# liuliu/ccv

Measured on AMD Instinct MI355X. Metric: images/sec fwd+bwd VGG-D 224x224 bs256, higher is better.
Workload: dtype f32 (Winograd-domain / fc GEMMs: exact bf16x3 split, all 9 products, fp32 accumulate); 1 GPU; VGG-D (ccv vgg_d_params, 225x225x3 crop, NHWC) forward+backward+SGD, batch 256 per GPU, random-init weights; global_batch=256, parallelism=dp1, conv_relu=convolution epilogue (NNC_MI355X_CONV_ALGO_FUSE_RELU)

## Files before the change

### ccv_amd/csrc/cmd_conv.cpp

```cpp
#include "gemm_launch.h"
#include "winograd.h"
#include "wino_fused.h"
#include "wino_wgrad_fused.h"
#include "conv_c3.h"

using namespace nnc;

namespace {

static size_t align256(size_t x) { return (x + 255) & ~(size_t)255; }

static thread_local int tl_relu_want = 0, tl_relu_done = 0;
static thread_local int tl_mask_want = 0, tl_mask_done = 0;
static thread_local Image4 tl_mask = { 0, 0, 0, 0, 0, 0, 0, 0, 0 };
static bool mask_fits(const Image4& dst)
{
	const Image4& m = tl_mask;
	return m.p && m.n == dst.n && m.h == dst.h && m.w == dst.w && m.c == dst.c && m.sc == 1 && aligned16(m.p) && m.sw % 4 == 0 && m.sh % 4 == 0 && (m.n == 1 || m.sn % 4 == 0);
}

struct back_share_t {
	int want_v;
	int want_bits;
	int GYn, GXn, KB;
	float* v;
	unsigned* bits;
	size_t v_off, bits_off;
};
static thread_local back_share_t tl_share = { 0, 0, 0, 0, 0, 0, 0, 0, 0 };

static void* g_dbg_bits_dst = 0;
static size_t g_dbg_bits_cap = 0, g_dbg_bits_got = 0;
static long g_back_shared[2] = { 0, 0 };

struct conv_geom_t {
	int N, H, W, C;
	int OH, OW, K;
	int kh, kw, Cg, Kg, groups;
	int sy, sx, pby, pbx, dy, dx;
};

static bool conv_geometry(const ccv_nnc_cmd_t& cmd, const ccv_nnc_hint_t& hint, const Image4& a, const Image4& b, const ccv_nnc_tensor_t* w, conv_geom_t* g)
{
	g->N = a.n; g->H = a.h; g->W = a.w; g->C = a.c;
	g->OH = b.h; g->OW = b.w; g->K = b.c;
	g->groups = cmd.info.convolution.groups > 0 ? cmd.info.convolution.groups : 1;
	g->kh = cmd.info.size.dim[0]; g->kw = cmd.info.size.dim[1];
	if (g->K != cmd.info.convolution.count || g->K % g->groups || g->C % g->groups || a.n != b.n) return false;
	g->Cg = g->C / g->groups; g->Kg = g->K / g->groups;
	g->sy = hint.stride.dim[0] > 0 ? hint.stride.dim[0] : 1;
	g->sx = hint.stride.dim[1] > 0 ? hint.stride.dim[1] : 1;
	g->pby = hint.border.begin[0]; g->pbx = hint.border.begin[1];
	g->dy = cmd.info.convolution.dilation[0] > 1 ? cmd.info.convolution.dilation[0] : 1;
	g->dx = cmd.info.convolution.dilation[1] > 1 ? cmd.info.convolution.dilation[1] : 1;
	(void)w;
	return true;
// ... 40 lines not shown
}

static int wino_slice_images(const int N, const int tiles_per_image, const int C_src, const int C_dst)
{
	const long kb = tune(TUNE_WINO_SLICE_KB);
	if (kb <= 0) return N;
	const double per_image = 36.0 * sizeof(float) * (double)tiles_per_image * (double)(C_src + C_dst);
	long nb = (long)((double)kb * 1024.0 / per_image);
	if (nb < 1) nb = 1;
	return nb > N ? N : (int)nb;
}

template <bool FLIP>
static int conv_wino_run(const char* name, const conv_geom_t& g, const wino_plan_t& p, const Image4& src, const float* w, const float* bias, const Image4& dst, const int pad_y, const int pad_x, const int flags, ccv_nnc_stream_context_t* const ctx)
{
	const int Cs = src.c, Cd = dst.c;
	const int per_image = p.TH * p.TW;
	const int nb = wino_slice_images(g.N, per_image, Cs, Cd);
	const size_t v_bytes = nb == g.N ? p.v_bytes : (sizeof(float) * 36 * (size_t)nb * per_image * Cs + 255) & ~(size_t)255;
	const size_t m_bytes = nb == g.N ? p.m_bytes : (sizeof(float) * 36 * (size_t)nb * per_image * Cd + 255) & ~(size_t)255;
	bool have_v = FLIP && tl_share.v && nb == g.N && p.u_bytes + m_bytes <= tl_share.v_off;
	size_t need = p.u_bytes + v_bytes + m_bytes;
	if (have_v && tl_share.v_off + v_bytes > need) need = tl_share.v_off + v_bytes;
	char* ws = (char*)workspace_of(ctx, need);
	if (!ws) return CCV_NNC_EXEC_OOM;
	if (have_v && (float*)(ws + tl_share.v_off) != tl_share.v) have_v = false;
	float* const U = (float*)ws;
	float* const V = have_v ? tl_share.v : (float*)(ws + p.u_bytes);
	float* const M = have_v ? (float*)(ws + p.u_bytes) : (float*)(ws + p.u_bytes + v_bytes);
	hipStream_t stream = stream_of(ctx);
	hipLaunchKernelGGL(HIP_KERNEL_NAME(wino_weight_kernel<FLIP>), dim3(blocks_exact((size_t)Cs * Cd, 256)), dim3(256), 0, stream, w, U, g.K, g.C);
	HIP_ENFORCE(hipGetLastError());
	for (int n0 = 0; n0 < g.N; n0 += nb) {
		const int ns = g.N - n0 < nb ? g.N - n0 : nb;
		const int T = ns * per_image;
		WinoTiles ti;
		ti.TH = p.TH; ti.TW = p.TW; ti.T = T;
		ti.H = src.h; ti.W = src.w; ti.sn = src.sn; ti.sh = src.sh; ti.sw = src.sw; ti.oy = -pad_y; ti.ox = -pad_x; ti.C4 = Cs / 4;
		ti.relu = (!FLIP && tl_relu_want) ? 1 : 0;
		if (ti.relu) tl_relu_done = 1;
		ti.mask = 0; ti.m_sn = ti.m_sh = ti.m_sw = 0;
		ti.d_c4.init(ti.C4); ti.d_tw.init(ti.TW); ti.d_th.init(ti.TH);
		if (!have_v) hipLaunchKernelGGL(HIP_KERNEL_NAME(wino_input_kernel<false>), dim3(blocks_exact((size_t)T * ti.C4, 256)), dim3(256), 0, stream, (const float*)src.p + (long)n0 * src.sn, V, ti, WinoMaskOut());
		HIP_ENFORCE(hipGetLastError());
		MatLoader<true, true> la, lb;
		la.p = V; la.ldr = Cs; la.ldk = 1; la.R = T; la.K = Cs;
		lb.p = U; lb.ldr = Cs; lb.ldk = 1; lb.R = Cd; lb.K = Cs;
		GemmOut out = { M, Cd, 1, 0, 1.f, 0 };
		const int ret = gemm_run(name, la, lb, out, T, Cd, Cs, 36, (long)T * Cs, (long)Cd * Cs, (long)T * Cd, 0L, 1, flags, ctx);
		if (ret != CCV_NNC_EXEC_SUCCESS) return ret;
		ti.H = dst.h; ti.W = dst.w; ti.sn = dst.sn; ti.sh = dst.sh; ti.sw = dst.sw; ti.C4 = Cd / 4;
		ti.d_c4.init(ti.C4);
		if (FLIP && mask_fits(dst)) {
			ti.mask = tl_mask.p + (long)n0 * tl_mask.sn; ti.m_sn = tl_mask.sn; ti.m_sh = tl_mask.sh; ti.m_sw = tl_mask.sw;
			tl_mask_done = 1;
		}
		hipLaunchKernelGGL(wino_output_kernel, dim3(blocks_exact((size_t)T * ti.C4, 256)), dim3(256), 0, stream, (const float*)M, bias, dst.p + (long)n0 * dst.sn, ti);
		HIP_ENFORCE(hipGetLastError());
	}
	return CCV_NNC_EXEC_SUCCESS;
}

struct wino_fused_plan_t {
	int GH, GW, GYn, GXn, groups, KB, CCn;
	size_t uf_bytes;
};

static bool wino_fused_plan(const conv_geom_t& g, const Image4& src, const Image4& dst, wino_fused_plan_t* p)
{
	if (g.kh != 3 || g.kw != 3 || g.sy != 1 || g.sx != 1 || g.dy != 1 || g.dx != 1 || g.groups != 1) return false;
	if (src.c % WF_CC || src.c < 2 * WF_CC || src.sc != 1 || dst.sc != 1 || !aligned16(src.p) || src.sw % 4 || src.sh % 4 || (src.n > 1 && src.sn % 4)) return false;
	if (dst.c % 4 || !aligned16(dst.p) || dst.sw % 4 || dst.sh % 4 || (dst.n > 1 && dst.sn % 4)) return false;
	if (((long)(dst.h - 1) * dst.sh + (long)(dst.w - 1) * dst.sw + dst.c) * 4 >= (long)WF_OOB) return false;
	if (((long)(src.h - 1) * src.sh + (long)(src.w - 1) * src.sw + src.c) * 4 >= (long)WF_OOB) return false;
	const int TH = (dst.h + 3) / 4, TW = (dst.w + 3) / 4;
	static const int shapes[3][2] = { { 4, 4 }, { 2, 8 }, { 8, 2 } };
	long best = -1;
	for (int i = 0; i < 3; i++) {
		const long cover = (long)((TH + shapes[i][0] - 1) / shapes[i][0]) * ((TW + shapes[i][1] - 1) / shapes[i][1]);
		if (best < 0 || cover < best) { best = cover; p->GH = shapes[i][0]; p->GW = shapes[i][1]; }
// ... 111 lines not shown
	const long tiles = (long)((g.K + 127) / 128) * ((g.C + 127) / 128) * 36;
	long s = ((long)device_cu_count() * 8 + tiles - 1) / tiles;
	const long max_s = p->t.T / (GEMM_BK * 8);
	if (s > max_s) s = max_s;
	if (s > 64) s = 64;
	p->splits = s <= 1 ? 1 : (int)(((s < 8 ? 8 : s) + 7) & ~7);
	p->w_bytes = p->t.m_bytes;
	p->du_bytes = (sizeof(float) * 36 * (size_t)g.K * g.C + 255) & ~(size_t)255;
	p->head_bytes = p->splits > 1 ? sizeof(float) * 36 * (size_t)g.K * g.C * p->splits : 0;
	const size_t colsum_bound = sizeof(float) * (size_t)device_cu_count() * 4 * g.K;
	if (p->head_bytes < colsum_bound) p->head_bytes = colsum_bound;
	p->head_bytes = (p->head_bytes + 255) & ~(size_t)255;
	p->blocks = ((long)p->t.T * (g.K / 4) + 255) / 256;
	p->bp_bytes = sizeof(float) * (size_t)p->blocks * g.K;
	return true;
}

static int conv_wino_wgrad(const conv_geom_t& g, const wino_wgrad_plan_t& p, const Image4& gr, const Image4& a, float* dw, float* dbias, bool* bias_done, const int flags, ccv_nnc_stream_context_t* const ctx)
{
	const int per_image = p.t.TH * p.t.TW;
	const int nb = wino_slice_images(g.N, per_image, g.C, g.K);
	const size_t bits_bytes = (size_t)g.N * tl_share.GYn * tl_share.GXn * tl_share.KB * 1024;
	const bool fuse_bias = dbias && 256 % (g.K / 4) == 0;
	const size_t extra = nb != g.N ? 0 : (tl_share.want_v ? (fuse_bias ? p.w_bytes : 0) : (tl_share.want_bits ? bits_bytes : 0));
	char* ws = (char*)workspace_of(ctx, p.total() + extra);
	if (!ws) return CCV_NNC_EXEC_OOM;
	float* const Vg = extra && tl_share.want_v ? (float*)(ws + p.total()) : 0;
	unsigned* const bits = extra && tl_share.want_bits ? (unsigned*)(ws + p.total()) : 0;
	float* const V = (float*)(ws + p.head_bytes);
	float* const W = (float*)(ws + p.head_bytes + p.t.v_bytes);
	float* const dU = (float*)(ws + p.head_bytes + p.t.v_bytes + p.w_bytes);
	float* const BP = (float*)(ws + p.head_bytes + p.t.v_bytes + p.w_bytes + p.du_bytes);
	const int acc = (flags & CCV_NNC_ACCUMULATE_OUTPUT) ? 1 : 0;
	hipStream_t stream = stream_of(ctx);
	if (bits && (tl_share.GYn * 2 != p.t.TH || tl_share.GXn * 8 != p.t.TW || g.C % WF_KT)) {
		const int r = fill_f32((float*)bits, bits_bytes / sizeof(float), 0.f, ctx);
		if (r != CCV_NNC_EXEC_SUCCESS) return r;
	}
	for (int n0 = 0; n0 < g.N; n0 += nb) {
		const int ns = g.N - n0 < nb ? g.N - n0 : nb;
		const int T = ns * per_image;
		WinoTiles ti;
		ti.TH = p.t.TH; ti.TW = p.t.TW; ti.T = T;
		ti.H = a.h; ti.W = a.w; ti.sn = a.sn; ti.sh = a.sh; ti.sw = a.sw; ti.oy = -g.pby; ti.ox = -g.pbx; ti.C4 = g.C / 4;
		ti.d_c4.init(ti.C4); ti.d_tw.init(ti.TW); ti.d_th.init(ti.TH);
		if (bits) {
			WinoMaskOut mo;
			mo.bits = (unsigned char*)bits; mo.GYn = tl_share.GYn; mo.GXn = tl_share.GXn; mo.KB = tl_share.KB;
			hipLaunchKernelGGL(HIP_KERNEL_NAME(wino_input_kernel<true>), dim3(blocks_exact((size_t)T * ti.C4, 256)), dim3(256), 0, stream, (const float*)a.p + (long)n0 * a.sn, V, ti, mo);
			tl_share.bits = bits; tl_share.bits_off = p.total();
			__atomic_fetch_add(&g_back_shared[1], 1L, __ATOMIC_RELAXED);
		} else hipLaunchKernelGGL(HIP_KERNEL_NAME(wino_input_kernel<false>), dim3(blocks_exact((size_t)T * ti.C4, 256)), dim3(256), 0, stream, (const float*)a.p + (long)n0 * a.sn, V, ti, WinoMaskOut());
		HIP_ENFORCE(hipGetLastError());
		ti.H = gr.h; ti.W = gr.w; ti.sn = gr.sn; ti.sh = gr.sh; ti.sw = gr.sw; ti.oy = 0; ti.ox = 0; ti.C4 = g.K / 4;
		ti.d_c4.init(ti.C4);
		const long blocks = ((long)T * (g.K / 4) + 255) / 256;
		const float* const grs = (const float*)gr.p + (long)n0 * gr.sn;
		if (Vg) {
			ti.oy = -1; ti.ox = -1;
			hipLaunchKernelGGL(wino_outgrad_both_kernel, dim3((unsigned)blocks), dim3(256), 0, stream, grs, Vg, W, ti, BP);
			tl_share.v = Vg; tl_share.v_off = p.total();
			__atomic_fetch_add(&g_back_shared[0], 1L, __ATOMIC_RELAXED);
		} else if (fuse_bias) hipLaunchKernelGGL(HIP_KERNEL_NAME(wino_outgrad_kernel<true>), dim3((unsigned)blocks), dim3(256), 0, stream, grs, W, ti, BP);
		else hipLaunchKernelGGL(HIP_KERNEL_NAME(wino_outgrad_kernel<false>), dim3((unsigned)blocks), dim3(256), 0, stream, grs, W, ti, (float*)0);
		HIP_ENFORCE(hipGetLastError());
		MatLoader<false, true> la, lb;
		la.p = W; la.ldr = 1; la.ldk = g.K; la.R = g.K; la.K = T;
		lb.p = V; lb.ldr = 1; lb.ldk = g.C; lb.R = g.C; lb.K = T;
		GemmOut out = { dU, g.C, 1, 0, 1.f, n0 > 0 ? 1 : 0 };
		int splits = p.splits;
		if (nb < g.N) {
			const long max_s = T / (GEMM_BK * 8);
			if (splits > max_s) splits = max_s <= 1 ? 1 : (int)(max_s & ~7L);
			if (splits < 8) splits = 1;
		}
// ... 262 lines not shown
				const int r = conv_forw_nhwc(q, gr, Fw, 0, ti, CONV_ALGO_IMPLICIT_GEMM, flags & ~CCV_NNC_ACCUMULATE_OUTPUT, ctx);
				if (r != CCV_NNC_EXEC_SUCCESS) return r;
			}
			hipLaunchKernelGGL(parity_scatter_kernel, dim3(grid_for(cells, 256)), dim3(256), 0, stream, (const float*)T, h.p, U, V, vec ? g.C / 4 : -g.C, h.sn, h.sh, h.sw, py, px, cells);
			HIP_ENFORCE(hipGetLastError());
		}
	return CCV_NNC_EXEC_SUCCESS;
}

static bool conv_dgrad_takes_fused(const conv_geom_t& g, const Image4& gr, const Image4& h, const int algo, wino_fused_plan_t* fp)
{
	return algo != CONV_ALGO_IMPLICIT_GEMM && algo != CONV_ALGO_WINOGRAD && g.pby <= 2 && g.pbx <= 2 && g.pby >= 0 && g.pbx >= 0 && wino_fused_plan(g, gr, h, fp) && (algo == CONV_ALGO_WINOGRAD_FUSED || wino_fused_preferred(g.K, *fp, h));
}
static bool conv_dgrad_takes_wino(const conv_geom_t& g, const Image4& gr, const float* w, const Image4& h, const int algo, wino_plan_t* wp)
{
	return algo != CONV_ALGO_IMPLICIT_GEMM && wino_plan(g, g.H, g.W, g.K, g.C, wp) && wino_images_ok(gr, h, w, 0) && (algo >= CONV_ALGO_WINOGRAD || wino_preferred(*wp, g.K, g.C));
}

static int conv_dgrad_nhwc(const conv_geom_t& g, const Image4& gr, const float* w, const Image4& h, const int algo, const int flags, ccv_nnc_stream_context_t* const ctx)
{
	if (gr.sc != 1 || !pixel_linear(h) || !image_fits_int(gr)) return CCV_NNC_EXEC_INVALID;
	wino_plan_t wp;
	wino_fused_plan_t fp;
	if (conv_dgrad_takes_fused(g, gr, h, algo, &fp)) {
		const int r = conv_wino_fused_run<true>("conv_dgrad_wino_fused", g, fp, gr, w, 0, h, 2 - g.pby, 2 - g.pbx, ctx);
		if (r != CCV_NNC_EXEC_OOM) return r;
	}
	if (conv_dgrad_takes_wino(g, gr, w, h, algo, &wp)) {
		const int r = conv_wino_run<true>("conv_dgrad_wino", g, wp, gr, w, 0, h, 2 - g.pby, 2 - g.pbx, flags, ctx);
		if (r != CCV_NNC_EXEC_OOM) return r;
	}
	if (algo != CONV_ALGO_IMPLICIT_GEMM && !(flags & CCV_NNC_ACCUMULATE_OUTPUT) && conv_dgrad_parity_ok(g) && g.kh * g.kw > 1) {
		const int r = conv_dgrad_parity(g, gr, w, h, flags, ctx);
		if (r != CCV_NNC_EXEC_OOM && r != CCV_NNC_EXEC_NO_KERNEL) return r;
	}
	const long M = (long)g.N * g.H * g.W;
	const int Kred = g.kh * g.kw * g.Kg;
	if (M > 0x7fffffffL) return CCV_NNC_EXEC_INVALID;
	const bool vec = (g.Kg % 4 == 0) && (g.Cg % 4 == 0) && aligned16(gr.p) && aligned16(w) && gr.sw % 4 == 0 && gr.sh % 4 == 0 && (gr.n == 1 || gr.sn % 4 == 0);
	GemmOut out = { h.p, h.sw, 1, 0, 1.f, 0 };
	if (vec && conv_pointwise(g, h, gr)) {
		MatLoader<true, true> la;
		la.p = gr.p; la.ldr = gr.sw; la.ldk = 1; la.R = (int)M; la.K = g.K;
		MatLoader<false, true> lb;
		lb.p = w; lb.ldr = 1; lb.ldk = g.C; lb.R = g.C; lb.K = g.K;
		return gemm_run("conv_dgrad_pointwise", la, lb, out, (int)M, g.C, g.K, 1, 0L, 0L, 0L, 0L, 1, flags, ctx);
	}
	KOrder ko;
	if (g.kh * g.kw > 1 && g.Kg % GEMM_BK == 0) ko.init(g.kh * g.kw, g.Kg);
#define CONV_DGRAD(VEC, STRIDED, INC) do { \
		Im2colKC<VEC, STRIDED, INC> la; \
		la.p = gr.p; la.s_n = gr.sn; la.s_h = (int)gr.sh; la.s_w = (int)gr.sw; la.H = g.OH; la.W = g.OW; \
// ... 239 lines not shown
	if (h && (!image4(h, &hi) || hi.h != g.H || hi.w != g.W || hi.c != g.C || hi.n != g.N || h->info.format != gt->info.format)) return CCV_NNC_EXEC_INVALID;
	if (dbias && (!tensor_contiguous(dbias) || dbias->info.dim[0] != g.K)) return CCV_NNC_EXEC_INVALID;
	const int acc = (flags & CCV_NNC_ACCUMULATE_OUTPUT) ? 1 : 0;
	const bool stage_io = gt->info.format == CCV_TENSOR_FORMAT_NCHW, stage_w = wshape->info.format == CCV_TENSOR_FORMAT_NCHW;
	const size_t wbytes = align256(sizeof(float) * (size_t)g.K * g.kh * g.kw * g.Cg);
	const size_t ng = stage_io ? align256(sizeof(float) * tensor_count(gt->info)) : 0;
	const size_t na = stage_io && a && dw ? align256(sizeof(float) * tensor_count(a->info)) : 0;
	const size_t nh = stage_io && h ? align256(sizeof(float) * tensor_count(h->info)) : 0;
	const size_t nw = stage_w && h ? wbytes : 0, ndw = stage_w && dw ? wbytes : 0;
	const long P = (long)g.N * g.OH * g.OW;
	size_t inner = gemm_workspace_bound(g.Kg, (long)g.kh * g.kw * g.Cg, P);
	const size_t inner_d = gemm_workspace_bound((long)g.N * g.H * g.W, g.Cg, (long)g.kh * g.kw * g.Kg), inner_b = sizeof(float) * (size_t)g.K * 4096;
	if (inner_d > inner) inner = inner_d;
	if (inner_b > inner) inner = inner_b;
	wino_plan_t wpl;
	if (h && cmd.algorithm != CONV_ALGO_IMPLICIT_GEMM && wino_plan(g, g.H, g.W, g.K, g.C, &wpl) && wpl.total() > inner) inner = wpl.total();
	wino_wgrad_plan_t wgp;
	if (dw && cmd.algorithm != CONV_ALGO_IMPLICIT_GEMM && wino_wgrad_plan(g, &wgp) && wgp.total() > inner) inner = wgp.total();
	wino_wgrad_fused_plan_t wfgp;
	if (dw && cmd.algorithm != CONV_ALGO_IMPLICIT_GEMM && wino_wgrad_fused_plan(g, &wfgp) && wfgp.total() > inner) inner = wfgp.total();
	if (h && cmd.algorithm != CONV_ALGO_IMPLICIT_GEMM && wino_fused_scratch_bound(g.C, g.K) + wino_fused_mask_bound(g) > inner) inner = wino_fused_scratch_bound(g.C, g.K) + wino_fused_mask_bound(g);
	if (h && cmd.algorithm != CONV_ALGO_IMPLICIT_GEMM && conv_dgrad_parity_scratch(g) > inner) inner = conv_dgrad_parity_scratch(g);
	if (dw && cmd.algorithm != CONV_ALGO_IMPLICIT_GEMM && g.C == 3 && conv_c3_wgrad_scratch_bound(g.K) > inner) inner = conv_c3_wgrad_scratch_bound(g.K);
	back_share_t share = { 0, 0, 0, 0, 0, 0, 0, 0, 0 };
	const long share_on = tune(TUNE_CONV_BACK_SHARE);
	if (h && dw && a && w && share_on && !stage_io && !stage_w && g.pby == 1 && g.pbx == 1 && g.OH == g.H && g.OW == g.W && ai.sc == 1 && gi.sc == 1 && pixel_linear(gi) && pixel_linear(hi) && image_fits_int(ai) && image_fits_int(gi)
		&& !(cmd.algorithm != CONV_ALGO_IMPLICIT_GEMM && conv_c3_ok(g, ai, gi))) {
		wino_wgrad_fused_plan_t wf;
		wino_wgrad_plan_t wg;
		wino_fused_plan_t fp;
		wino_plan_t wp;
		if (!conv_wgrad_takes_fused(g, gi, ai, dw->data.f32, cmd.algorithm, &wf) && conv_wgrad_takes_wino(g, gi, ai, dw->data.f32, cmd.algorithm, &wg) && wino_slice_images(g.N, wg.t.TH * wg.t.TW, g.C, g.K) == g.N) {
			if (conv_dgrad_takes_fused(g, gi, hi, cmd.algorithm, &fp)) {
				tl_mask = ai;
				if ((share_on & 2) && tl_mask_want && fp.GH == 2 && mask_fits(hi) && (long)fp.groups * fp.KB <= 0x7fffffffL && fp.uf_bytes <= wg.total()) {
					share.want_bits = 1; share.GYn = fp.GYn; share.GXn = fp.GXn; share.KB = fp.KB;
					if (wg.total() + (size_t)fp.groups * fp.KB * 1024 > inner) inner = wg.total() + (size_t)fp.groups * fp.KB * 1024;
				}
				tl_mask.p = 0;
			} else if ((share_on & 1) && dbias && 256 % (g.K / 4) == 0 && conv_dgrad_takes_wino(g, gi, w->data.f32, hi, cmd.algorithm, &wp) && wp.TH == wg.t.TH && wp.TW == wg.t.TW && wp.u_bytes + wp.m_bytes <= wg.total()) {
				share.want_v = 1;
				if (wg.total() + wg.w_bytes > inner) inner = wg.total() + wg.w_bytes;
			}
		}
	}
	struct share_scope_t { share_scope_t(const back_share_t& s) { tl_share = s; } ~share_scope_t() { const back_share_t none = { 0, 0, 0, 0, 0, 0, 0, 0, 0 }; tl_share = none; } } share_scope(share);
	WorkspaceScope ws(stream_context, ng + na + nh + nw + ndw, inner);
	char* p = (char*)ws.prefix();
	if ((ng + na + nh + nw + ndw) && !p) return CCV_NNC_EXEC_OOM;
	int ret;
	ccv_nnc_tensor_t gs, as, hs;
	Image4 gim = gi, aim = ai, him = hi;
	if (stage_io) {
		dense_nhwc_like(gt, gi, (float*)p, &gs);
		if ((ret = format_transform(gt, &gs, stream_context)) != CCV_NNC_EXEC_SUCCESS) return ret;
		image4(&gs, &gim);
		if (na) {
			dense_nhwc_like(a, ai, (float*)(p + ng), &as);
			if ((ret = format_transform(a, &as, stream_context)) != CCV_NNC_EXEC_SUCCESS) return ret;
			image4(&as, &aim);
		}
		if (nh) { dense_nhwc_like(h, hi, (float*)(p + ng + na), &hs); image4(&hs, &him); }
	}
	bool bias_done = false;
	if (dw) {
		float* dwp = dw->data.f32;
		if (stage_w) {
			dwp = (float*)(p + ng + na + nh + nw);
			if (acc && (ret = weights_nchw_to_nhwc(dw->data.f32, dwp, g.K, g.Cg, g.kh * g.kw, stream_context)) != CCV_NNC_EXEC_SUCCESS) return ret;
// ... 470 lines not shown
	const int trial_flags = flags & ~CCV_NNC_ACCUMULATE_OUTPUT;
	for (int algo = 0; algo < CONV_ALGO_COUNT; algo++) {
		ccv_nnc_cmd_t c = cmd;
		c.algorithm = algo;
		float ms = 0;
		int ok = 1;
		for (int trial = 0; trial < 2 && ok; trial++) {
			HIP_ENFORCE(hipEventRecord(e0, stream));
			const int ret = fwd ? _conv_forw(c, hint, trial_flags, inputs, input_size, outputs, output_size, stream_context) : _conv_back(c, hint, trial_flags, inputs, input_size, outputs, output_size, stream_context);
			HIP_ENFORCE(hipEventRecord(e1, stream));
			HIP_ENFORCE(hipEventSynchronize(e1));
			if (ret != CCV_NNC_EXEC_SUCCESS) ok = 0;
			else HIP_ENFORCE(hipEventElapsedTime(&ms, e0, e1));
		}
		if (ok && (!have_best || ms < best_ms)) { best = algo; best_ms = ms; have_best = 1; }
	}
	HIP_ENFORCE(hipEventDestroy(e0));
	HIP_ENFORCE(hipEventDestroy(e1));
	return best;
}

}

extern "C" long nnc_mi355x_debug_conv_back_shared(int what) { return what == 0 || what == 1 ? __atomic_load_n(&g_back_shared[what], __ATOMIC_RELAXED) : 0; }
extern "C" size_t nnc_mi355x_debug_conv_mask_bits(void* dst, size_t capacity)
{
	g_dbg_bits_dst = dst; g_dbg_bits_cap = capacity;
	return g_dbg_bits_got;
}

extern "C" void _register_command_CCV_NNC_CONVOLUTION_FORWARD_backend_CCV_NNC_BACKEND_GPU_CUDNN(ccv_nnc_cmd_backend_registry_t* const registry)
{
	registry->tensor_formats = CCV_TENSOR_FORMAT_NCHW | CCV_TENSOR_FORMAT_NHWC;
	registry->tensor_datatypes = CCV_32F | CCV_16F;
	registry->tensor_memory = CCV_TENSOR_GPU_MEMORY;
	registry->algorithms = CONV_ALGO_COUNT;
	registry->exec = _conv_forw_any;
	registry->autotune = _conv_autotune;
	NNC_DEPALETTIZED(registry, _conv_forw_any);
}

extern "C" void _register_command_CCV_NNC_CONVOLUTION_BACKWARD_backend_CCV_NNC_BACKEND_GPU_CUDNN(ccv_nnc_cmd_backend_registry_t* const registry)
{
	registry->tensor_formats = CCV_TENSOR_FORMAT_NCHW | CCV_TENSOR_FORMAT_NHWC;
	registry->tensor_datatypes = CCV_32F | CCV_16F;
	registry->tensor_memory = CCV_TENSOR_GPU_MEMORY;
	registry->algorithms = CONV_ALGO_COUNT;
// ... 16 lines not shown
```

### ccv_amd/csrc/common.h

```cpp
#pragma once
#include <hip/hip_runtime.h>
#include <atomic>
#include <stdio.h>
#include <stdlib.h>
#include <string.h>
#include <assert.h>
#include "../../include/nnc_mi355x.h"

#define HIP_ENFORCE(expr) do { \
	const hipError_t _st = (expr); \
	if (_st != hipSuccess) { \
		fprintf(stderr, "[%s:%d]:HIP - Error: %d (%s)\n", __FILE__, __LINE__, (int)_st, hipGetErrorString(_st)); \
		abort(); \
	} \
} while (0)

extern "C" void* nnc_staging_of(const ccv_nnc_stream_context_t* stream_context, size_t size);
extern "C" void* nnc_palette_of(const ccv_nnc_stream_context_t* stream_context, size_t size);

namespace nnc {

static inline int tensor_nd(const int dim[CCV_NNC_MAX_DIM_ALLOC])
{
	int i;
// ... 175 lines not shown
extern int g_force_tile;
extern int g_force_splits;

enum {
	TUNE_WINO_SLICE_KB = 0,
	TUNE_WINO_FUSED_MAX_C,
	TUNE_WINO_FUSED_GRID,
	TUNE_GRID_WG_PER_CU,
	TUNE_WINO_WGRAD_FUSED_MAX,
	TUNE_GEMM_BUFFER_LOADS,
	TUNE_CONV_NCHW_HALF_F16,
	TUNE_BN_SMALL_PLANES,
	TUNE_SDPA_MFMA,
	TUNE_BN_CLUSTER,
	TUNE_GEMM_VEC_EPILOGUE,
	TUNE_POOL_ROWS,
	TUNE_GEMM_HALF_CHUNK8,
	TUNE_LSTM_PERSISTENT,
	TUNE_LSTM_ROWS,
	TUNE_GEMM_BF16X3,
	TUNE_BN_CLUSTER_SLOTS,
	TUNE_GEMM_BATCH_XCD,
	TUNE_CONV_BACK_SHARE,
	TUNE_COUNT
};
static_assert(TUNE_GRID_WG_PER_CU == 3, "grid_for() above names this key by value");
long tune(int key);

constexpr int FOLD_CH = 16, FOLD_PH = 16;
__device__ __forceinline__ float fold_slices(const float* __restrict__ p, const long slices, const int C, const int c, const int phase)
{
	float s0 = 0.f, s1 = 0.f, s2 = 0.f, s3 = 0.f;
	long i = phase;
	for (; i + 3 * FOLD_PH < slices; i += 4 * FOLD_PH) {
		s0 += p[i * C + c]; s1 += p[(i + FOLD_PH) * C + c]; s2 += p[(i + 2 * FOLD_PH) * C + c]; s3 += p[(i + 3 * FOLD_PH) * C + c];
	}
	for (; i < slices; i += FOLD_PH) s0 += p[i * C + c];
	return (s0 + s1) + (s2 + s3);
}
__device__ __forceinline__ float fold_phases(float (*red)[FOLD_CH], const int ch)
{
	float a[FOLD_PH];
#pragma unroll
	for (int k = 0; k < FOLD_PH; k++) a[k] = red[k][ch];
#pragma unroll
	for (int w = FOLD_PH / 2; w >= 1; w >>= 1)
// ... 35 lines not shown
```

### ccv_amd/csrc/device_rt.cpp

```cpp
#include "common.h"
#include <atomic>
#include <pthread.h>
#include <dlfcn.h>
#include <vector>
#include <list>
#include <deque>
#include <mutex>
#include <unordered_map>

namespace {

struct device_local_t {
	hipStream_t stream;
	void* workspace;
	size_t workspace_size;
	int device;
	void* staging;
	size_t staging_size;
	void* palette;
	size_t palette_size;
	void* cluster_sync;
	unsigned cluster_epoch;
	unsigned long cluster_capture;
	unsigned long capture_alias;
// ... 82 lines not shown
		memset(s->any + s->any_size, 0, sizeof(device_local_t) * (device + 1 - s->any_size));
		s->any_size = device + 1;
	}
	device_local_t* l = s->any + device;
	if (!l->stream) {
		l->device = device;
		HIP_ENFORCE(hipStreamCreateWithFlags(&l->stream, hipStreamDefault));
		pool_stream_created(device, l->stream);
	}
	return l;
}

inline hipStream_t effective_stream(device_local_t* const l)
{
	if (g_capture_active.load(std::memory_order_acquire) > 0 && l->capture_alias == g_capture_id.load(std::memory_order_acquire) && l->capture_alias && l->device >= 0 && l->device < CAP_MAX_DEVICES && g_cap_rep[l->device]) return g_cap_rep[l->device];
	return l->stream;
}

}

namespace nnc {
int g_force_tile = 0;
int g_force_splits = 0;
static const char* const g_tune_names[TUNE_COUNT] = { "WINO_SLICE_KB", "WINO_FUSED_MAX_C", "WINO_FUSED_GRID", "GRID_WG_PER_CU", "WINO_WGRAD_FUSED_MAX", "GEMM_BUFFER_LOADS", "CONV_NCHW_HALF_F16", "BN_SMALL_PLANES", "SDPA_MFMA", "BN_CLUSTER", "GEMM_VEC_EPILOGUE", "POOL_ROWS", "GEMM_HALF_CHUNK8", "LSTM_PERSISTENT", "LSTM_ROWS", "GEMM_BF16X3", "BN_CLUSTER_SLOTS", "GEMM_BATCH_XCD", "CONV_BACK_SHARE" };
static long g_tune_values[TUNE_COUNT] = { 0, 128, 0, 0, 128, 1, 32, 1, 1, 1, 1, 1, 1, 1, 1, 1, 0, 1, 3 };
static int g_tune_env_read = 0;
long tune(int key)
{
	if (!g_tune_env_read) {
		for (int i = 0; i < TUNE_COUNT; i++) {
			char name[64];
			snprintf(name, sizeof(name), "NNC_MI355X_%s", g_tune_names[i]);
			const char* v = getenv(name);
			if (v && *v) g_tune_values[i] = atol(v);
		}
		g_tune_env_read = 1;
	}
	return key >= 0 && key < TUNE_COUNT ? g_tune_values[key] : 0;
}
}
namespace nnc {

static inline device_local_t* joined(device_local_t* const l)
{
	if (g_comm_overlap_epoch.load(std::memory_order_acquire) != l->comm_seen) comm_overlap_join(l->stream, &l->comm_seen);
	return l;
}
std::atomic<unsigned long> g_launch_seq(0);
// ... 1226 lines not shown
```

### ccv_amd/csrc/winograd.h

```cpp
#pragma once
#include "mfma_gemm.h"

namespace nnc {

template <class T>
__device__ __forceinline__ void wino_bt(const T (&x)[6], T (&y)[6])
{
	const T a = x[4] - 4.f * x[2], b = x[3] - 4.f * x[1];
	const T c = x[4] - x[2], d = 2.f * (x[3] - x[1]);
	y[0] = 4.f * x[0] - 5.f * x[2] + x[4];
	y[1] = a + b;
	y[2] = a - b;
	y[3] = c + d;
	y[4] = c - d;
	y[5] = 4.f * x[1] - 5.f * x[3] + x[5];
}
template <class T>
__device__ __forceinline__ void wino_g(const T (&x)[3], T (&y)[6])
{
	const T s = x[0] + x[2];
	const T e = x[0] * (1.f / 24.f) + x[2] * (1.f / 6.f), o = x[1] * (1.f / 12.f);
	y[0] = x[0] * 0.25f;
	y[1] = (s + x[1]) * (-1.f / 6.f);
	y[2] = (s - x[1]) * (-1.f / 6.f);
// ... 65 lines not shown
		float y[6];
		wino_g(col, y);
#pragma unroll
		for (int i = 0; i < 6; i++) t[i][j] = y[i];
	}
	const long plane = (long)R * Q;
#pragma unroll
	for (int i = 0; i < 6; i++) {
		float y[6];
		wino_g(t[i], y);
#pragma unroll
		for (int j = 0; j < 6; j++) u[(long)(i * 6 + j) * plane + idx] = y[j];
	}
}

struct WinoTiles {
	int TH, TW, T;
	int H, W;
	long sn, sh, sw;
	int oy, ox;
	int C4;
	int relu;
	const float* mask; long m_sn, m_sh, m_sw;
	FastDiv d_c4, d_tw, d_th;
};

constexpr int WINO_MASK_KT = 32;
__host__ __device__ __forceinline__ long wino_mask_item(const long n, const int gy, const int gx, const int kb, const int GYn, const int GXn, const int KB) { return ((n * GYn + gy) * GXn + gx) * KB + kb; }
__host__ __device__ __forceinline__ int wino_mask_pid(const int e, const int lane) { return e * 8 + (lane >> 3); }
__host__ __device__ __forceinline__ int wino_mask_tile(const int pid, const int r) { return 4 * (pid >> 4) + r; }
__host__ __device__ __forceinline__ int wino_mask_round(const int tile) { return tile & 3; }
__host__ __device__ __forceinline__ int wino_mask_pid_of(const int tile, const int px) { return 16 * (tile >> 2) + px; }
__host__ __device__ __forceinline__ int wino_mask_nibble(const int pid) { return pid >> 3; }
__host__ __device__ __forceinline__ int wino_mask_lane(const int pid, const int q8) { return (pid & 7) * 8 + q8; }

struct WinoMaskOut {
	unsigned char* bits;
	int GYn, GXn, KB;
};

template <bool MASK>
static __global__ void __launch_bounds__(256) wino_input_kernel(const float* __restrict__ a, float* __restrict__ v, const WinoTiles g, const WinoMaskOut mo)
{
	const long idx = (long)nnc_xcd_block(blockIdx.x, gridDim.x) * blockDim.x + threadIdx.x;
	if (idx >= (long)g.T * g.C4) return;
	const int t = g.d_c4.div((int)idx), c4 = (int)(idx - (long)t * g.C4);
	const int tn = g.d_tw.div(t), tx = t - tn * g.TW;
	const int n = g.d_th.div(tn), ty = tn - n * g.TH;
	const int y0 = ty * 4 + g.oy, x0 = tx * 4 + g.ox;
	const float* const src = a + (long)n * g.sn + (long)c4 * 4;
	f4 s[6][6];
	unsigned mb[8];
#pragma unroll
	for (int r = 0; r < 6; r++) {
		const int y = y0 + r;
		const bool yok = (y >= 0) & (y < g.H);
		f4 d[6];
#pragma unroll
		for (int q = 0; q < 6; q++) {
			const int x = x0 + q;
			const bool ok = yok & (x >= 0) & (x < g.W);
			d[q] = ok ? f4(*(const float4*)(src + (long)y * g.sh + (long)x * g.sw)) : f4(0.f, 0.f, 0.f, 0.f);
		}
		if (MASK && r >= 1 && r <= 4) {
#pragma unroll
			for (int q = 0; q < 4; q++) {
				const f4 m = d[q + 1];
				const unsigned nib = (m.x > 0.f ? 1u : 0u) | (m.y > 0.f ? 2u : 0u) | (m.z > 0.f ? 4u : 0u) | (m.w > 0.f ? 8u : 0u);
				const int px = 4 * (r - 1) + q;
				if (px < 8) mb[px] = nib; else mb[px - 8] |= nib << 4;
			}
		}
		wino_bt(d, s[r]);
	}
	if (MASK) {
		const int gy = ty >> 1, gx = tx >> 3, tile = (ty & 1) * 8 + (tx & 7);
		const long item = wino_mask_item(n, gy, gx, c4 >> 3, mo.GYn, mo.GXn, mo.KB);
		unsigned char* const bp = mo.bits + (item * 256 + wino_mask_round(tile) * 64) * 4;
#pragma unroll
		for (int j = 0; j < 8; j++) {
			const int pid = wino_mask_pid_of(tile, j);
			bp[wino_mask_lane(pid, c4 & 7) * 4 + (wino_mask_nibble(pid) >> 1)] = (unsigned char)mb[j];
		}
	}
	const long plane = (long)g.T * g.C4 * 4;
	float* const dst = v + idx * 4;
#pragma unroll
	for (int q = 0; q < 6; q++) {
		const f4 col[6] = { s[0][q], s[1][q], s[2][q], s[3][q], s[4][q], s[5][q] };
		f4 y[6];
		wino_bt(col, y);
#pragma unroll
		for (int r = 0; r < 6; r++) *(float4*)(dst + (long)(r * 6 + q) * plane) = y[r];
	}
}

static __global__ void __launch_bounds__(256) wino_output_kernel(const float* __restrict__ m, const float* __restrict__ bias, float* __restrict__ b, const WinoTiles g)
{
	const long idx = (long)blockIdx.x * blockDim.x + threadIdx.x;
	if (idx >= (long)g.T * g.C4) return;
	const int t = g.d_c4.div((int)idx), k4 = (int)(idx - (long)t * g.C4);
	const int tn = g.d_tw.div(t), tx = t - tn * g.TW;
	const int n = g.d_th.div(tn), ty = tn - n * g.TH;
	const long plane = (long)g.T * g.C4 * 4;
	const float* const src = m + idx * 4;
	f4 s[4][6];
#pragma unroll
	for (int q = 0; q < 6; q++) {
		f4 col[6];
#pragma unroll
		for (int r = 0; r < 6; r++) col[r] = f4(*(const float4*)(src + (long)(r * 6 + q) * plane));
		f4 y[4];
		wino_at(col, y);
#pragma unroll
		for (int i = 0; i < 4; i++) s[i][q] = y[i];
	}
	const f4 bv = bias ? f4(*(const float4*)(bias + k4 * 4)) : f4(0.f, 0.f, 0.f, 0.f);
	float* const dst = b + (long)n * g.sn + (long)k4 * 4;
	const float* const msk = g.mask ? g.mask + (long)n * g.m_sn + (long)k4 * 4 : 0;
#pragma unroll
	for (int i = 0; i < 4; i++) {
		f4 y[4];
		wino_at(s[i], y);
		const int oy = ty * 4 + i;
#pragma unroll
		for (int j = 0; j < 4; j++) {
			const int ox = tx * 4 + j;
			if ((oy < g.H) & (ox < g.W)) {
				f4 o = y[j] + bv;
				if (g.relu) o = f4(fmaxf(o.x, 0.f), fmaxf(o.y, 0.f), fmaxf(o.z, 0.f), fmaxf(o.w, 0.f));
				if (msk) {
					const float4 mv = *(const float4*)(msk + (long)oy * g.m_sh + (long)ox * g.m_sw);
					o = f4(mv.x > 0.f ? o.x : 0.f, mv.y > 0.f ? o.y : 0.f, mv.z > 0.f ? o.z : 0.f, mv.w > 0.f ? o.w : 0.f);
				}
				*(float4*)(dst + (long)oy * g.sh + (long)ox * g.sw) = (float4)o;
			}
		}
	}
}

template <bool COLSUM>
static __global__ void __launch_bounds__(256) wino_outgrad_kernel(const float* __restrict__ gr, float* __restrict__ wt, const WinoTiles g, float* __restrict__ blockpart)
{
	__shared__ float4 red[COLSUM ? 256 : 1];
	const long idx = (long)blockIdx.x * blockDim.x + threadIdx.x;
	const bool live = idx < (long)g.T * g.C4;
	f4 sum(0.f, 0.f, 0.f, 0.f);
	if (live) {
		const int t = g.d_c4.div((int)idx), k4 = (int)(idx - (long)t * g.C4);
		const int tn = g.d_tw.div(t), tx = t - tn * g.TW;
		const int n = g.d_th.div(tn), ty = tn - n * g.TH;
		const float* const src = gr + (long)n * g.sn + (long)k4 * 4;
		f4 s[4][6];
#pragma unroll
		for (int r = 0; r < 4; r++) {
			const int y = ty * 4 + r;
			f4 d[4];
#pragma unroll
			for (int q = 0; q < 4; q++) {
				const int x = tx * 4 + q;
				const bool ok = (y < g.H) & (x < g.W);
// ... 121 lines not shown
```

Measured before the change: 3466 images/s.

## Route large-K dgrad through shared-V Winograd GEMM with packed ReLU mask words

For layers whose K exceeds the fused-Winograd limit, conv backward now prefers the unfused Winograd dgrad path. That path reuses the input-transform V already computed by the wgrad pass, so the dgrad input transform is skipped. The wgrad input kernel also emits a 64-bit per-tile ReLU mask word, which the dgrad output kernel reads in place of the full float activation mask. The aim is to cut redundant transform work and mask memory traffic. In exchange the code uses more workspace and changes the algorithm choice for these layers, and the GEMM path may be slower than the fused kernel it replaces.

```diff
diff --git a/ccv_amd/csrc/cmd_conv.cpp b/ccv_amd/csrc/cmd_conv.cpp
--- a/ccv_amd/csrc/cmd_conv.cpp
+++ b/ccv_amd/csrc/cmd_conv.cpp
@@ -26,12 +26,16 @@
 	float* v;
 	unsigned* bits;
 	size_t v_off, bits_off;
+	int want_words;
+	int dgrad_gemm;
+	unsigned long long* words;
+	size_t words_off;
 };
-static thread_local back_share_t tl_share = { 0, 0, 0, 0, 0, 0, 0, 0, 0 };
+static thread_local back_share_t tl_share = {};
 
 static void* g_dbg_bits_dst = 0;
 static size_t g_dbg_bits_cap = 0, g_dbg_bits_got = 0;
-static long g_back_shared[2] = { 0, 0 };
+static long g_back_shared[3] = { 0, 0, 0 };
 
 struct conv_geom_t {
 	int N, H, W, C;
@@ -118,9 +122,13 @@
 	bool have_v = FLIP && tl_share.v && nb == g.N && p.u_bytes + m_bytes <= tl_share.v_off;
 	size_t need = p.u_bytes + v_bytes + m_bytes;
 	if (have_v && tl_share.v_off + v_bytes > need) need = tl_share.v_off + v_bytes;
+	const size_t words_bytes = sizeof(unsigned long long) * (size_t)p.T * (Cd / 4);
+	bool have_words = have_v && tl_share.words && mask_fits(dst);
+	if (have_words && tl_share.words_off + words_bytes > need) need = tl_share.words_off + words_bytes;
 	char* ws = (char*)workspace_of(ctx, need);
 	if (!ws) return CCV_NNC_EXEC_OOM;
 	if (have_v && (float*)(ws + tl_share.v_off) != tl_share.v) have_v = false;
+	if (have_words && (!have_v || (unsigned long long*)(ws + tl_share.words_off) != tl_share.words)) have_words = false;
 	float* const U = (float*)ws;
 	float* const V = have_v ? tl_share.v : (float*)(ws + p.u_bytes);
 	float* const M = have_v ? (float*)(ws + p.u_bytes) : (float*)(ws + p.u_bytes + v_bytes);
@@ -135,9 +143,9 @@
 		ti.H = src.h; ti.W = src.w; ti.sn = src.sn; ti.sh = src.sh; ti.sw = src.sw; ti.oy = -pad_y; ti.ox = -pad_x; ti.C4 = Cs / 4;
 		ti.relu = (!FLIP && tl_relu_want) ? 1 : 0;
 		if (ti.relu) tl_relu_done = 1;
-		ti.mask = 0; ti.m_sn = ti.m_sh = ti.m_sw = 0;
+		ti.mask = 0; ti.m_sn = ti.m_sh = ti.m_sw = 0; ti.mwords = 0;
 		ti.d_c4.init(ti.C4); ti.d_tw.init(ti.TW); ti.d_th.init(ti.TH);
-		if (!have_v) hipLaunchKernelGGL(HIP_KERNEL_NAME(wino_input_kernel<false>), dim3(blocks_exact((size_t)T * ti.C4, 256)), dim3(256), 0, stream, (const float*)src.p + (long)n0 * src.sn, V, ti, WinoMaskOut());
+		if (!have_v) hipLaunchKernelGGL(HIP_KERNEL_NAME(wino_input_kernel<0>), dim3(blocks_exact((size_t)T * ti.C4, 256)), dim3(256), 0, stream, (const float*)src.p + (long)n0 * src.sn, V, ti, WinoMaskOut());
 		HIP_ENFORCE(hipGetLastError());
 		MatLoader<true, true> la, lb;
 		la.p = V; la.ldr = Cs; la.ldk = 1; la.R = T; la.K = Cs;
@@ -149,9 +157,11 @@
 		ti.d_c4.init(ti.C4);
 		if (FLIP && mask_fits(dst)) {
 			ti.mask = tl_mask.p + (long)n0 * tl_mask.sn; ti.m_sn = tl_mask.sn; ti.m_sh = tl_mask.sh; ti.m_sw = tl_mask.sw;
+			if (have_words) ti.mwords = tl_share.words;
 			tl_mask_done = 1;
 		}
-		hipLaunchKernelGGL(wino_output_kernel, dim3(blocks_exact((size_t)T * ti.C4, 256)), dim3(256), 0, stream, (const float*)M, bias, dst.p + (long)n0 * dst.sn, ti);
+		if (ti.mwords) hipLaunchKernelGGL(wino_output_bits_kernel, dim3(blocks_exact((size_t)T * ti.C4, 256)), dim3(256), 0, stream, (const float*)M, bias, dst.p + (long)n0 * dst.sn, ti);
+		else hipLaunchKernelGGL(wino_output_kernel, dim3(blocks_exact((size_t)T * ti.C4, 256)), dim3(256), 0, stream, (const float*)M, bias, dst.p + (long)n0 * dst.sn, ti);
 		HIP_ENFORCE(hipGetLastError());
 	}
 	return CCV_NNC_EXEC_SUCCESS;
@@ -309,10 +319,12 @@
 	const int nb = wino_slice_images(g.N, per_image, g.C, g.K);
 	const size_t bits_bytes = (size_t)g.N * tl_share.GYn * tl_share.GXn * tl_share.KB * 1024;
 	const bool fuse_bias = dbias && 256 % (g.K / 4) == 0;
-	const size_t extra = nb != g.N ? 0 : (tl_share.want_v ? (fuse_bias ? p.w_bytes : 0) : (tl_share.want_bits ? bits_bytes : 0));
+	const size_t words_bytes = tl_share.want_v && tl_share.want_words ? align256(sizeof(unsigned long long) * (size_t)p.t.T * (g.C / 4)) : 0;
+	const size_t extra = nb != g.N ? 0 : (tl_share.want_v ? (fuse_bias ? p.w_bytes + words_bytes : 0) : (tl_share.want_bits ? bits_bytes : 0));
 	char* ws = (char*)workspace_of(ctx, p.total() + extra);
 	if (!ws) return CCV_NNC_EXEC_OOM;
 	float* const Vg = extra && tl_share.want_v ? (float*)(ws + p.total()) : 0;
+	unsigned long long* const words = Vg && words_bytes ? (unsigned long long*)(ws + p.total() + p.w_bytes) : 0;
 	unsigned* const bits = extra && tl_share.want_bits ? (unsigned*)(ws + p.total()) : 0;
 	float* const V = (float*)(ws + p.head_bytes);
 	float* const W = (float*)(ws + p.head_bytes + p.t.v_bytes);
@@ -333,11 +345,17 @@
 		ti.d_c4.init(ti.C4); ti.d_tw.init(ti.TW); ti.d_th.init(ti.TH);
 		if (bits) {
 			WinoMaskOut mo;
-			mo.bits = (unsigned char*)bits; mo.GYn = tl_share.GYn; mo.GXn = tl_share.GXn; mo.KB = tl_share.KB;
-			hipLaunchKernelGGL(HIP_KERNEL_NAME(wino_input_kernel<true>), dim3(blocks_exact((size_t)T * ti.C4, 256)), dim3(256), 0, stream, (const float*)a.p + (long)n0 * a.sn, V, ti, mo);
+			mo.bits = (unsigned char*)bits; mo.GYn = tl_share.GYn; mo.GXn = tl_share.GXn; mo.KB = tl_share.KB; mo.words = 0;
+			hipLaunchKernelGGL(HIP_KERNEL_NAME(wino_input_kernel<1>), dim3(blocks_exact((size_t)T * ti.C4, 256)), dim3(256), 0, stream, (const float*)a.p + (long)n0 * a.sn, V, ti, mo);
 			tl_share.bits = bits; tl_share.bits_off = p.total();
 			__atomic_fetch_add(&g_back_shared[1], 1L, __ATOMIC_RELAXED);
-		} else hipLaunchKernelGGL(HIP_KERNEL_NAME(wino_input_kernel<false>), dim3(blocks_exact((size_t)T * ti.C4, 256)), dim3(256), 0, stream, (const float*)a.p + (long)n0 * a.sn, V, ti, WinoMaskOut());
+		} else if (words) {
+			WinoMaskOut mo;
+			mo.bits = 0; mo.GYn = mo.GXn = mo.KB = 0; mo.words = words;
+			hipLaunchKernelGGL(HIP_KERNEL_NAME(wino_input_kernel<2>), dim3(blocks_exact((size_t)T * ti.C4, 256)), dim3(256), 0, stream, (const float*)a.p + (long)n0 * a.sn, V, ti, mo);
+			tl_share.words = words; tl_share.words_off = p.total() + p.w_bytes;
+			__atomic_fetch_add(&g_back_shared[2], 1L, __ATOMIC_RELAXED);
+		} else hipLaunchKernelGGL(HIP_KERNEL_NAME(wino_input_kernel<0>), dim3(blocks_exact((size_t)T * ti.C4, 256)), dim3(256), 0, stream, (const float*)a.p + (long)n0 * a.sn, V, ti, WinoMaskOut());
 		HIP_ENFORCE(hipGetLastError());
 		ti.H = gr.h; ti.W = gr.w; ti.sn = gr.sn; ti.sh = gr.sh; ti.sw = gr.sw; ti.oy = 0; ti.ox = 0; ti.C4 = g.K / 4;
 		ti.d_c4.init(ti.C4);
@@ -646,12 +664,17 @@
 	if (gr.sc != 1 || !pixel_linear(h) || !image_fits_int(gr)) return CCV_NNC_EXEC_INVALID;
 	wino_plan_t wp;
 	wino_fused_plan_t fp;
-	if (conv_dgrad_takes_fused(g, gr, h, algo, &fp)) {
+	const bool gemm_first = tl_share.dgrad_gemm && tl_share.v;
+	if (!gemm_first && conv_dgrad_takes_fused(g, gr, h, algo, &fp)) {
 		const int r = conv_wino_fused_run<true>("conv_dgrad_wino_fused", g, fp, gr, w, 0, h, 2 - g.pby, 2 - g.pbx, ctx);
 		if (r != CCV_NNC_EXEC_OOM) return r;
 	}
 	if (conv_dgrad_takes_wino(g, gr, w, h, algo, &wp)) {
 		const int r = conv_wino_run<true>("conv_dgrad_wino", g, wp, gr, w, 0, h, 2 - g.pby, 2 - g.pbx, flags, ctx);
+		if (r != CCV_NNC_EXEC_OOM) return r;
+	}
+	if (gemm_first && conv_dgrad_takes_fused(g, gr, h, algo, &fp)) {
+		const int r = conv_wino_fused_run<true>("conv_dgrad_wino_fused", g, fp, gr, w, 0, h, 2 - g.pby, 2 - g.pbx, ctx);
 		if (r != CCV_NNC_EXEC_OOM) return r;
 	}
 	if (algo != CONV_ALGO_IMPLICIT_GEMM && !(flags & CCV_NNC_ACCUMULATE_OUTPUT) && conv_dgrad_parity_ok(g) && g.kh * g.kw > 1) {
@@ -937,7 +960,7 @@
 	if (h && cmd.algorithm != CONV_ALGO_IMPLICIT_GEMM && wino_fused_scratch_bound(g.C, g.K) + wino_fused_mask_bound(g) > inner) inner = wino_fused_scratch_bound(g.C, g.K) + wino_fused_mask_bound(g);
 	if (h && cmd.algorithm != CONV_ALGO_IMPLICIT_GEMM && conv_dgrad_parity_scratch(g) > inner) inner = conv_dgrad_parity_scratch(g);
 	if (dw && cmd.algorithm != CONV_ALGO_IMPLICIT_GEMM && g.C == 3 && conv_c3_wgrad_scratch_bound(g.K) > inner) inner = conv_c3_wgrad_scratch_bound(g.K);
-	back_share_t share = { 0, 0, 0, 0, 0, 0, 0, 0, 0 };
+	back_share_t share = {};
 	const long share_on = tune(TUNE_CONV_BACK_SHARE);
 	if (h && dw && a && w && share_on && !stage_io && !stage_w && g.pby == 1 && g.pbx == 1 && g.OH == g.H && g.OW == g.W && ai.sc == 1 && gi.sc == 1 && pixel_linear(gi) && pixel_linear(hi) && image_fits_int(ai) && image_fits_int(gi)
 		&& !(cmd.algorithm != CONV_ALGO_IMPLICIT_GEMM && conv_c3_ok(g, ai, gi))) {
@@ -946,20 +969,30 @@
 		wino_fused_plan_t fp;
 		wino_plan_t wp;
 		if (!conv_wgrad_takes_fused(g, gi, ai, dw->data.f32, cmd.algorithm, &wf) && conv_wgrad_takes_wino(g, gi, ai, dw->data.f32, cmd.algorithm, &wg) && wino_slice_images(g.N, wg.t.TH * wg.t.TW, g.C, g.K) == g.N) {
-			if (conv_dgrad_takes_fused(g, gi, hi, cmd.algorithm, &fp)) {
+			const auto v_shareable = [&]() { return (share_on & 1) && dbias && 256 % (g.K / 4) == 0 && conv_dgrad_takes_wino(g, gi, w->data.f32, hi, cmd.algorithm, &wp) && wp.TH == wg.t.TH && wp.TW == wg.t.TW && wp.u_bytes + wp.m_bytes <= wg.total(); };
+			const auto want_v = [&]() {
+				share.want_v = 1;
+				size_t most = wg.total() + wg.w_bytes;
+				tl_mask = ai;
+				if ((share_on & 4) && tl_mask_want && mask_fits(hi)) { share.want_words = 1; most += align256(sizeof(unsigned long long) * (size_t)wg.t.T * (g.C / 4)); }
+				tl_mask.p = 0;
+				if (most > inner) inner = most;
+			};
+			const bool fused = conv_dgrad_takes_fused(g, gi, hi, cmd.algorithm, &fp);
+			if (fused && tune(TUNE_CONV_BACK_DGRAD_GEMM) && cmd.algorithm != CONV_ALGO_WINOGRAD_FUSED && g.K > tune(TUNE_WINO_FUSED_MAX_C) && v_shareable()) {
+				share.dgrad_gemm = 1;
+				want_v();
+			} else if (fused) {
 				tl_mask = ai;
 				if ((share_on & 2) && tl_mask_want && fp.GH == 2 && mask_fits(hi) && (long)fp.groups * fp.KB <= 0x7fffffffL && fp.uf_bytes <= wg.total()) {
 					share.want_bits = 1; share.GYn = fp.GYn; share.GXn = fp.GXn; share.KB = fp.KB;
 					if (wg.total() + (size_t)fp.groups * fp.KB * 1024 > inner) inner = wg.total() + (size_t)fp.groups * fp.KB * 1024;
 				}
 				tl_mask.p = 0;
-			} else if ((share_on & 1) && dbias && 256 % (g.K / 4) == 0 && conv_dgrad_takes_wino(g, gi, w->data.f32, hi, cmd.algorithm, &wp) && wp.TH == wg.t.TH && wp.TW == wg.t.TW && wp.u_bytes + wp.m_bytes <= wg.total()) {
-				share.want_v = 1;
-				if (wg.total() + wg.w_bytes > inner) inner = wg.total() + wg.w_bytes;
-			}
+			} else if (v_shareable()) want_v();
 		}
 	}
-	struct share_scope_t { share_scope_t(const back_share_t& s) { tl_share = s; } ~share_scope_t() { const back_share_t none = { 0, 0, 0, 0, 0, 0, 0, 0, 0 }; tl_share = none; } } share_scope(share);
+	struct share_scope_t { share_scope_t(const back_share_t& s) { tl_share = s; } ~share_scope_t() { const back_share_t none = {}; tl_share = none; } } share_scope(share);
 	WorkspaceScope ws(stream_context, ng + na + nh + nw + ndw, inner);
 	char* p = (char*)ws.prefix();
 	if ((ng + na + nh + nw + ndw) && !p) return CCV_NNC_EXEC_OOM;
@@ -1476,7 +1509,7 @@
 
 }
 
-extern "C" long nnc_mi355x_debug_conv_back_shared(int what) { return what == 0 || what == 1 ? __atomic_load_n(&g_back_shared[what], __ATOMIC_RELAXED) : 0; }
+extern "C" long nnc_mi355x_debug_conv_back_shared(int what) { return what >= 0 && what <= 2 ? __atomic_load_n(&g_back_shared[what], __ATOMIC_RELAXED) : 0; }
 extern "C" size_t nnc_mi355x_debug_conv_mask_bits(void* dst, size_t capacity)
 {
 	g_dbg_bits_dst = dst; g_dbg_bits_cap = capacity;
diff --git a/ccv_amd/csrc/common.h b/ccv_amd/csrc/common.h
--- a/ccv_amd/csrc/common.h
+++ b/ccv_amd/csrc/common.h
@@ -221,6 +221,7 @@
 	TUNE_BN_CLUSTER_SLOTS,
 	TUNE_GEMM_BATCH_XCD,
 	TUNE_CONV_BACK_SHARE,
+	TUNE_CONV_BACK_DGRAD_GEMM,
 	TUNE_COUNT
 };
 static_assert(TUNE_GRID_WG_PER_CU == 3, "grid_for() above names this key by value");
diff --git a/ccv_amd/csrc/device_rt.cpp b/ccv_amd/csrc/device_rt.cpp
--- a/ccv_amd/csrc/device_rt.cpp
+++ b/ccv_amd/csrc/device_rt.cpp
@@ -128,8 +128,8 @@
 namespace nnc {
 int g_force_tile = 0;
 int g_force_splits = 0;
-static const char* const g_tune_names[TUNE_COUNT] = { "WINO_SLICE_KB", "WINO_FUSED_MAX_C", "WINO_FUSED_GRID", "GRID_WG_PER_CU", "WINO_WGRAD_FUSED_MAX", "GEMM_BUFFER_LOADS", "CONV_NCHW_HALF_F16", "BN_SMALL_PLANES", "SDPA_MFMA", "BN_CLUSTER", "GEMM_VEC_EPILOGUE", "POOL_ROWS", "GEMM_HALF_CHUNK8", "LSTM_PERSISTENT", "LSTM_ROWS", "GEMM_BF16X3", "BN_CLUSTER_SLOTS", "GEMM_BATCH_XCD", "CONV_BACK_SHARE" };
-static long g_tune_values[TUNE_COUNT] = { 0, 128, 0, 0, 128, 1, 32, 1, 1, 1, 1, 1, 1, 1, 1, 1, 0, 1, 3 };
+static const char* const g_tune_names[TUNE_COUNT] = { "WINO_SLICE_KB", "WINO_FUSED_MAX_C", "WINO_FUSED_GRID", "GRID_WG_PER_CU", "WINO_WGRAD_FUSED_MAX", "GEMM_BUFFER_LOADS", "CONV_NCHW_HALF_F16", "BN_SMALL_PLANES", "SDPA_MFMA", "BN_CLUSTER", "GEMM_VEC_EPILOGUE", "POOL_ROWS", "GEMM_HALF_CHUNK8", "LSTM_PERSISTENT", "LSTM_ROWS", "GEMM_BF16X3", "BN_CLUSTER_SLOTS", "GEMM_BATCH_XCD", "CONV_BACK_SHARE", "CONV_BACK_DGRAD_GEMM" };
+static long g_tune_values[TUNE_COUNT] = { 0, 128, 0, 0, 128, 1, 32, 1, 1, 1, 1, 1, 1, 1, 1, 1, 0, 1, 7, 1 };
 static int g_tune_env_read = 0;
 long tune(int key)
 {
diff --git a/ccv_amd/csrc/winograd.h b/ccv_amd/csrc/winograd.h
--- a/ccv_amd/csrc/winograd.h
+++ b/ccv_amd/csrc/winograd.h
@@ -111,6 +111,7 @@
 	int C4;
 	int relu;
 	const float* mask; long m_sn, m_sh, m_sw;
+	const unsigned long long* mwords;
 	FastDiv d_c4, d_tw, d_th;
 };
 
@@ -126,9 +127,10 @@
 struct WinoMaskOut {
 	unsigned char* bits;
 	int GYn, GXn, KB;
+	unsigned long long* words;
 };
 
-template <bool MASK>
+template <int MASK>
 static __global__ void __launch_bounds__(256) wino_input_kernel(const float* __restrict__ a, float* __restrict__ v, const WinoTiles g, const WinoMaskOut mo)
 {
 	const long idx = (long)nnc_xcd_block(blockIdx.x, gridDim.x) * blockDim.x + threadIdx.x;
@@ -140,6 +142,7 @@
 	const float* const src = a + (long)n * g.sn + (long)c4 * 4;
 	f4 s[6][6];
 	unsigned mb[8];
+	unsigned long long mw = 0;
 #pragma unroll
 	for (int r = 0; r < 6; r++) {
 		const int y = y0 + r;
@@ -157,12 +160,14 @@
 				const f4 m = d[q + 1];
 				const unsigned nib = (m.x > 0.f ? 1u : 0u) | (m.y > 0.f ? 2u : 0u) | (m.z > 0.f ? 4u : 0u) | (m.w > 0.f ? 8u : 0u);
 				const int px = 4 * (r - 1) + q;
-				if (px < 8) mb[px] = nib; else mb[px - 8] |= nib << 4;
+				if (MASK == 2) mw |= (unsigned long long)nib << (4 * px);
+				else if (px < 8) mb[px] = nib; else mb[px - 8] |= nib << 4;
 			}
 		}
 		wino_bt(d, s[r]);
 	}
-	if (MASK) {
+	if (MASK == 2) mo.words[idx] = mw;
+	else if (MASK) {
 		const int gy = ty >> 1, gx = tx >> 3, tile = (ty & 1) * 8 + (tx & 7);
 		const long item = wino_mask_item(n, gy, gx, c4 >> 3, mo.GYn, mo.GXn, mo.KB);
 		unsigned char* const bp = mo.bits + (item * 256 + wino_mask_round(tile) * 64) * 4;
@@ -184,7 +189,8 @@
 	}
 }
 
-static __global__ void __launch_bounds__(256) wino_output_kernel(const float* __restrict__ m, const float* __restrict__ bias, float* __restrict__ b, const WinoTiles g)
+template <bool BITS>
+static __device__ __forceinline__ void wino_output_body(const float* __restrict__ m, const float* __restrict__ bias, float* __restrict__ b, const WinoTiles& g)
 {
 	const long idx = (long)blockIdx.x * blockDim.x + threadIdx.x;
 	if (idx >= (long)g.T * g.C4) return;
@@ -206,7 +212,8 @@
 	}
 	const f4 bv = bias ? f4(*(const float4*)(bias + k4 * 4)) : f4(0.f, 0.f, 0.f, 0.f);
 	float* const dst = b + (long)n * g.sn + (long)k4 * 4;
-	const float* const msk = g.mask ? g.mask + (long)n * g.m_sn + (long)k4 * 4 : 0;
+	const float* const msk = !BITS && g.mask ? g.mask + (long)n * g.m_sn + (long)k4 * 4 : 0;
+	const unsigned long long mw = BITS ? g.mwords[idx] : 0;
 #pragma unroll
 	for (int i = 0; i < 4; i++) {
 		f4 y[4];
@@ -218,7 +225,10 @@
 			if ((oy < g.H) & (ox < g.W)) {
 				f4 o = y[j] + bv;
 				if (g.relu) o = f4(fmaxf(o.x, 0.f), fmaxf(o.y, 0.f), fmaxf(o.z, 0.f), fmaxf(o.w, 0.f));
-				if (msk) {
+				if (BITS) {
+					const unsigned nib = (unsigned)(mw >> (4 * (4 * i + j))) & 15u;
+					o = f4((nib & 1u) ? o.x : 0.f, (nib & 2u) ? o.y : 0.f, (nib & 4u) ? o.z : 0.f, (nib & 8u) ? o.w : 0.f);
+				} else if (msk) {
 					const float4 mv = *(const float4*)(msk + (long)oy * g.m_sh + (long)ox * g.m_sw);
 					o = f4(mv.x > 0.f ? o.x : 0.f, mv.y > 0.f ? o.y : 0.f, mv.z > 0.f ? o.z : 0.f, mv.w > 0.f ? o.w : 0.f);
 				}
@@ -226,6 +236,14 @@
 			}
 		}
 	}
+}
+static __global__ void __launch_bounds__(256) wino_output_kernel(const float* __restrict__ m, const float* __restrict__ bias, float* __restrict__ b, const WinoTiles g)
+{
+	wino_output_body<false>(m, bias, b, g);
+}
+static __global__ void __launch_bounds__(256) wino_output_bits_kernel(const float* __restrict__ m, const float* __restrict__ bias, float* __restrict__ b, const WinoTiles g)
+{
+	wino_output_body<true>(m, bias, b, g);
 }
 
 template <bool COLSUM>
```

Measured after the change: 3499 images/s, median of 6. Within noise of the previous version (+0.9%).
